# PKU-EPIC/HOTrack

Hardware: AMD Instinct MI355X
Metric: HandTrackNet point-cloud frames/sec (N=1024) (higher is better)
Workload: dtype f32; 1 GPU; HandTrackNet forward, batch=64 synthetic 1024-pt clouds per GPU (BASELINE configs[1]); per_gpu_batch=64, global_batch=64, npoints=1024, parallelism=dp1 (independent batches, no collective), world_size=1, resident_batches_rotated=5, dead_attention_elided=True, fused_sa_kernels=True, launch=hipGraph replay, batches_in_flight=4, hip_hw_queues=4, sa_compute_units=256, weights=deterministic random init (no checkpoint available offline)

## Files before the change

### hotrack_amd/csrc/sa_fused.hip

```cpp
#include <stdlib.h>

#include "pn2_common.h"
#include "../../include/pn2_ext.h"

#ifndef SA_PAD
#define SA_PAD 4
#endif

#ifndef SA_DEFER_EPILOGUE
#define SA_DEFER_EPILOGUE 0
#endif
#ifndef SA_OVERLAP_WRITEOUT
#define SA_OVERLAP_WRITEOUT 1
#endif
#ifndef SA_SCALAR_L1
#define SA_SCALAR_L1 0
#endif
#ifndef SA_LOADER_PRIO
#define SA_LOADER_PRIO 0
#endif
#ifndef SA_PROBE
#define SA_PROBE 0
#endif
#ifndef SA_PREFETCH
// ... 54 lines not shown
}

struct SaArgs {
    int B, N, S, K, lgK;
    const float *a1f;
    const float *xyz;
    const float *cxyz;
    const float *wx;
    const float *b1;
    const float *cadd;
    int a1f_ld, cadd_ld;
    const int *idx;
    const float *w2, *b2, *w3, *b3;
    const float *w2e;
    float *out;
    long out_b;
    int out_s, out_c;
    int num_tiles, tiles_per_cloud;
    long long *trace;
    const int *cls_list;
    const int *cls_sizes;
};

template <int C1, int C2, int C3, int WC, int RTC, int MINW, int NB1, int K, int MODE>
__device__ __forceinline__ void sa_body(const SaArgs &A, const int wg, const int nwg) {
    static_assert(K == 0 || K == 16 || K == 32 || K == 64, "K");
    constexpr bool CLS = K == 0;
    constexpr bool ROWS = MODE == 4 || MODE == 5, ROWS_EXTRA = MODE == 5;
    static_assert(!ROWS_EXTRA || SA_PAD >= 4, "the extra input columns live in the LDS row padding");
    constexpr bool has_a1f = MODE >= 1, has_xyz = !ROWS, has_cadd = MODE == 2 || MODE == 3;
    const bool p_a1f = MODE == 3 ? A.a1f != nullptr : has_a1f, p_xyz = MODE == 3 ? A.xyz != nullptr : has_xyz;
    const bool p_cadd = MODE == 3 ? A.cadd != nullptr : has_cadd;
    constexpr int lgK = K == 16 ? 4 : K == 32 ? 5 : 6;
    const int N = A.N, S = A.S;
    const float *__restrict__ W2 = A.w2, *__restrict__ b2 = A.b2, *__restrict__ W3 = A.w3, *__restrict__ b3 = A.b3;
    float *__restrict__ out = A.out;
    const int num_tiles = A.num_tiles, tiles_per_cloud = A.tiles_per_cloud;
    constexpr int WP = 4 / WC;
    constexpr int TM = WP * 64;
    constexpr int LD1 = C1 + SA_PAD, LD2 = C2 + SA_PAD;
    constexpr int NT2 = C2 / (16 * WC), NT3 = C3 / (16 * WC);
    static_assert(C2 % (16 * WC) == 0 && C3 % (16 * WC) == 0 && C1 % 16 == 0, "tile geometry");
    extern __shared__ __attribute__((aligned(16))) float smem[];
    float *H1ring = smem;
    float *H2 = smem + NB1 * TM * LD1;

    const int tid = (int)__builtin_amdgcn_workitem_id_x();
    const int lane = tid & 63;
    const int w = tid >> 6;
// ... 329 lines not shown
            }
#endif
            stamp(it, 4);
#if !(SA_PROBE & 2)
            if (nx.tile < end) finish(D1, H1n, 1);
#endif
            stamp(it, 5);
            __syncthreads();
            stamp(it, 6);
            nx = af;
            af = CLS ? ag : cursor_next(af);
            if constexpr (CLS) ag = cursor_next(ag);
        }
        return;
    }
#ifdef SA_COMPUTE_PRIO
    __builtin_amdgcn_s_setprio(SA_COMPUTE_PRIO);
#endif
    int it = 0;
    Cursor cc = cursor_at(first);
    constexpr int NP = 4 / RTC, NQ2 = C1 / 16, NQ3 = C2 / 16;
    constexpr int rstep = CLS ? 4 : K >> 4;
    const int oc_lane = (wc * NT3 + g) * 16 + li;
    const unsigned out_cloud = 4u * ((unsigned)(S - 1) * (unsigned)A.out_s + (unsigned)(C3 - 1) * (unsigned)A.out_c + 1u);
    const rsrc_t ro_rows = make_rsrc(out, ROWS ? 4u * (unsigned)N * (unsigned)A.out_s : 0u);
    float m[4][NT3];
#pragma unroll
    for (int rt = 0; rt < 4; ++rt)
#pragma unroll
        for (int ct = 0; ct < NT3; ++ct) m[rt][ct] = 0.f;
    int e_b = 0, e_pos0 = 0;
    bool e_pending = false;
    auto epilogue = [&]() {
        if constexpr (K == 32) {
#pragma unroll
            for (int ct = 0; ct < NT3; ++ct) {
                m[0][ct] = fmax_raw(m[0][ct], m[1][ct]);
                m[2][ct] = fmax_raw(m[2][ct], m[3][ct]);
            }
        }
        if constexpr (K == 64) {
#pragma unroll
            for (int ct = 0; ct < NT3; ++ct) m[0][ct] = fmax_raw(fmax3_raw(m[0][ct], m[1][ct], m[2][ct]), m[3][ct]);
        }
        const rsrc_t ro = make_rsrc(out + (size_t)e_b * A.out_b, e_pending ? out_cloud : 0u);
#pragma unroll
        for (int rt = 0; rt < 4; rt += rstep) {
            const int s = ((e_pos0 + wp * 64) >> lgK) + rt / rstep;
#pragma unroll
            for (int ct0 = 0; ct0 < NT3; ct0 += 4) {
                float v = rows_max4(m[rt][ct0]);
#pragma unroll
                for (int j = 1; j < 4; ++j)
                    if (ct0 + j < NT3) {
                        const float vj = rows_max4(m[rt][ct0 + j]);
                        v = g == j ? vj : v;
                    }
                const unsigned off = 4u * ((unsigned)s * (unsigned)A.out_s + (unsigned)(oc_lane + 16 * ct0) * (unsigned)A.out_c);
                const bool ok = ct0 + g < NT3 && s < S;
                __builtin_amdgcn_raw_buffer_store_b32(__builtin_bit_cast(unsigned, fmaxf(v, 0.f)), ro, (int)(ok ? off : 0xffffffffu), 0, 0);
            }
        }
    };
    int me_b = 0, me_s = 0;
    auto load_me = [&](const Cursor &cu) {
        const int lgk = 5 - cu.b;
        const int n_c = sel3(cu.b, cls_n0, cls_n1, cls_n2), off = sel3(cu.b, 0, cls_n0, cls_n0 + cls_n1);
        const rsrc_t rl = make_rsrc(A.cls_list + 4 * (size_t)off, 16u * (unsigned)n_c);
        const unsigned slot = ((unsigned)(cu.t * TM + wp * 64) >> lgk) + (unsigned)(lane & 7);
        const i32x2 v = __builtin_bit_cast(i32x2, __builtin_amdgcn_raw_buffer_load_b64(rl, (int)(16u * slot + 8u), 0, 0));
        me_b = v.x; me_s = v.y;
    };
    const unsigned out_all = 4u * ((unsigned)(A.B - 1) * (unsigned)A.out_b + (unsigned)(S - 1) * (unsigned)A.out_s + (unsigned)(C3 - 1) * (unsigned)A.out_c + 1u);
    auto epilogue_cls = [&](const Cursor &cu) {
        static_assert(!CLS || NT3 == 2, "class walk: a lane row stores one of two channel tiles");
        const int lgk = 5 - cu.b;
        const int n_c = sel3(cu.b, cls_n0, cls_n1, cls_n2);
        const int slot0 = (int)((unsigned)(cu.t * TM + wp * 64) >> lgk);
        const rsrc_t ro = make_rsrc(out, out_all);
        auto store = [&](float v, int src, int ct, bool lane_ok) {
            const unsigned bb = (unsigned)__builtin_amdgcn_ds_bpermute(4 * src, me_b), ss = (unsigned)__builtin_amdgcn_ds_bpermute(4 * src, me_s);
            const unsigned off = 4u * (bb * (unsigned)A.out_b + ss * (unsigned)A.out_s + (unsigned)((wc * NT3 + ct) * 16 + li) * (unsigned)A.out_c);
// ... 181 lines not shown

template <int C1, int C2, int C3, int WC, int RTC, int MINW, int NB1, int K, int MODE>
__global__ void __launch_bounds__(512, MINW)
sa_mlp_max_kernel(const SaArgs A, const int grid) {
    sa_body<C1, C2, C3, WC, RTC, MINW, NB1, K, MODE>(A, (int)__builtin_amdgcn_workgroup_id_x(), grid);
}

template <int C1, int C2, int C3, int WC, int RTC, int MINW, int NB1, int MODE>
__global__ void __launch_bounds__(512, MINW)
sa_mlp_max_classes_kernel(const SaArgs A, const int grid) {
    sa_body<C1, C2, C3, WC, RTC, MINW, NB1, 0, MODE>(A, (int)__builtin_amdgcn_workgroup_id_x(), grid);
}

template <int C1, int C2, int C3, int WC, int RTC, int MINW, int NB1, int K0, int K1, int MODE>
__global__ void __launch_bounds__(512, MINW)
sa_mlp_max_pair_kernel(const SaArgs A0, const SaArgs A1, const int n0, const int n1) {
    const int wg = (int)__builtin_amdgcn_workgroup_id_x();
    if (wg < n0)
        sa_body<C1, C2, C3, WC, RTC, MINW, NB1, K0, MODE>(A0, wg, n0);
    else
        sa_body<C1, C2, C3, WC, RTC, MINW, NB1, K1, MODE>(A1, wg - n0, n1);
}

static int g_sa_cus = -1;
static int sa_compute_units() {
    if (g_sa_cus < 0) {
        const char *e = getenv("PN2_SA_CUS");
        g_sa_cus = e ? atoi(e) : 0;
    }
    const int all = num_compute_units();
    return (g_sa_cus > 0 && g_sa_cus < all) ? g_sa_cus : all;
}

constexpr int sa_tile_rows(int WC) { return (4 / WC) * 64; }

static int sa_set_tiles(SaArgs &a, int tm) {
    a.tiles_per_cloud = (a.S * a.K + tm - 1) / tm;
    const long num_tiles = (long)a.B * a.tiles_per_cloud;
    if (num_tiles > 2147483647L) return PN2_ERANGE;
    a.num_tiles = (int)num_tiles;
    a.lgK = 0;
    while ((1 << a.lgK) < a.K) ++a.lgK;
    return PN2_OK;
}

static int sa_grid_rounds(int tiles, int max_wg) {
// ... 13 lines not shown
static int sa_grid_classes(long centroids, int tm, long max_wg) {
    const long most = (centroids * 32 + tm - 1) / tm + 2;
    return (int)(most < max_wg ? most : max_wg);
}

template <auto kfn, int C1, int C2, int WC, int MINW, int NB1>
static int sa_launch_shape(size_t &lds) {
    lds = (size_t)sa_tile_rows(WC) * (NB1 * (C1 + SA_PAD) + C2 + SA_PAD) * sizeof(float);
    static PerDeviceOnce raised;
    if (lds > 64 * 1024 && raised.first_use())
        (void)hipFuncSetAttribute((const void *)kfn, hipFuncAttributeMaxDynamicSharedMemorySize, (int)lds);
    const int wg_per_cu = (int)((160 * 1024) / lds) < MINW / 2 ? (int)((160 * 1024) / lds) : MINW / 2;
    return sa_compute_units() * (wg_per_cu < 1 ? 1 : wg_per_cu);
}

template <int C1, int C2, int C3, int WC, int RTC, int MINW, int NB1, int K, int MODE>
static int launch_sa_km(SaArgs a, hipStream_t st) {
    if (sa_set_tiles(a, sa_tile_rows(WC)) != PN2_OK) return PN2_ERANGE;
    constexpr auto kfn = sa_mlp_max_kernel<C1, C2, C3, WC, RTC, MINW, NB1, K, MODE>;
    size_t lds;
    const int max_wg = sa_launch_shape<kfn, C1, C2, WC, MINW, NB1>(lds);
    const int grid = sa_grid_rounds(a.num_tiles, max_wg);
    hipLaunchKernelGGL(kfn, dim3(grid), dim3(512), lds, st, a, grid);
    return check_launch();
}

template <int C1, int C2, int C3, int WC, int RTC, int MINW, int NB1, int MODE>
static int launch_sa_classes(SaArgs a, hipStream_t st) {
    a.lgK = 5; a.tiles_per_cloud = 1;
    constexpr auto kfn = sa_mlp_max_classes_kernel<C1, C2, C3, WC, RTC, MINW, NB1, MODE>;
    size_t lds;
    const int max_wg = sa_launch_shape<kfn, C1, C2, WC, MINW, NB1>(lds);
    const int grid = sa_grid_classes((long)a.B * a.S, sa_tile_rows(WC), max_wg);
    hipLaunchKernelGGL(kfn, dim3(grid), dim3(512), lds, st, a, grid);
    return check_launch();
}

template <int C1, int C2, int C3, int WC, int RTC, int MINW, int NB1, int K0, int K1, int MODE>
static int launch_sa_pair(SaArgs a0, SaArgs a1, hipStream_t st) {
    if (sa_set_tiles(a0, sa_tile_rows(WC)) != PN2_OK || sa_set_tiles(a1, sa_tile_rows(WC)) != PN2_OK ||
        (long)a0.num_tiles + a1.num_tiles > 2147483647L)
        return PN2_ERANGE;
    constexpr auto kfn = sa_mlp_max_pair_kernel<C1, C2, C3, WC, RTC, MINW, NB1, K0, K1, MODE>;
    size_t lds;
    const int max_wg = sa_launch_shape<kfn, C1, C2, WC, MINW, NB1>(lds);
    int n0, n1;
    sa_grid_pair(a0.num_tiles, a1.num_tiles, max_wg, n0, n1);
    hipLaunchKernelGGL(kfn, dim3(n0 + n1), dim3(512), lds, st, a0, a1, n0, n1);
    return check_launch();
}

static int sa_mode(const SaArgs &a) {
    const bool fa = a.a1f != nullptr, fx = a.xyz != nullptr, fc = a.cadd != nullptr;
    if (!fx || (fc && !fa)) return 3;
    return fa ? (fc ? 2 : 1) : 0;
}

template <int C1, int C2, int C3, int WC, int RTC, int MINW, int NB1, int K>
static int launch_sa_k(const SaArgs &a, hipStream_t st) {
    switch (sa_mode(a)) {
        case 0: return launch_sa_km<C1, C2, C3, WC, RTC, MINW, NB1, K, 0>(a, st);
        case 1: return launch_sa_km<C1, C2, C3, WC, RTC, MINW, NB1, K, 1>(a, st);
        case 2: return launch_sa_km<C1, C2, C3, WC, RTC, MINW, NB1, K, 2>(a, st);
    }
    return launch_sa_km<C1, C2, C3, WC, RTC, MINW, NB1, K, 3>(a, st);
}

template <int C1, int C2, int C3, int WC, int RTC, int MINW, int NB1>
static int launch_sa(const SaArgs &a, hipStream_t st) {
    switch (a.K) {
        case 16: return launch_sa_k<C1, C2, C3, WC, RTC, MINW, NB1, 16>(a, st);
// ... 219 lines not shown
}

extern "C" int pn2x_sa_mlp_max_pair_supported(int k0, int k1, int c1, int c2, int c3) {
    return (c1 == 128 && c2 == 128 && c3 == 192 && ((k0 == 16 && k1 == 64) || (k0 == 64 && k1 == 16))) ? 1 : 0;
}

static_assert(sizeof(pn2x_sa_problem) == 144, "record layout (pn2_ext.h)");
extern "C" int pn2x_sa_mlp_max_pair(int b, int c1, int c2, int c3, const pn2x_sa_problem *p0, const pn2x_sa_problem *p1, void *stream) {
    using namespace pn2;
    if (b < 0 || !p0 || !p1) return b < 0 ? PN2_EINVAL : PN2_ENULL;
    if (b == 0) return PN2_OK;
    if (!pn2x_sa_mlp_max_pair_supported(p0->k, p1->k, c1, c2, c3)) return PN2_ERANGE;
    if (p0->k > p1->k) { const pn2x_sa_problem *t = p0; p0 = p1; p1 = t; }
    SaArgs a0, a1;
    if (const int rc = sa_check_fill(b, *p0, c1, c3, a0); rc != PN2_OK) return rc;
    if (const int rc = sa_check_fill(b, *p1, c1, c3, a1); rc != PN2_OK) return rc;
    const int mode = sa_mode(a0);
    if (mode != sa_mode(a1) || (mode != 1 && mode != 2)) return PN2_ERANGE;
    hipStream_t st = (hipStream_t)stream;
    if (mode == 2) return launch_sa_pair<128, 128, 192, 4, SA_RTC128, 2, SA_NB1, 16, 64, 2>(a0, a1, st);
    return launch_sa_pair<128, 128, 192, 4, SA_RTC128, 2, SA_NB1, 16, 64, 1>(a0, a1, st);
}

extern "C" int pn2x_mlp2_rows_supported(int c1, int c2, int c3) { return (c1 == 128 && c2 == 128 && c3 == 128) ? 1 : 0; }

extern "C" int pn2x_mlp2_rows(long rows, int c1, int c2, int c3, const float *x, int ldx, const float *w2, const float *w2e, const float *b2,
                              const float *w3, const float *b3, float *out, int ldo, void *stream) {
    using namespace pn2;
    if (rows < 0 || ldx < c1 + (w2e ? 4 : 0) || ldo < c3 || ldx % 4 || ldo % 4) return PN2_EINVAL;
    if (rows == 0) return PN2_OK;
    if (!x || !w2 || !b2 || !w3 || !b3 || !out) return PN2_ENULL;
    if (!pn2x_mlp2_rows_supported(c1, c2, c3)) return PN2_ERANGE;
    if (((uintptr_t)x | (uintptr_t)w2 | (uintptr_t)w3 | (uintptr_t)out) % 16 != 0) return PN2_EINVAL;
    if (rows >= (1L << 24) - 64 || 4L * ldx >= (1L << 24) || 4L * rows * ldx > 0xffffffffL || 4L * rows * ldo > 0xffffffffL) return PN2_ERANGE;
    SaArgs a = {};
    a.B = 1; a.N = (int)rows; a.K = 16; a.S = (int)((rows + 15) / 16);
    a.a1f = x; a.a1f_ld = ldx; a.w2 = w2; a.b2 = b2; a.w3 = w3; a.b3 = b3; a.w2e = w2e; a.out = out; a.out_s = ldo; a.out_c = 1;
    if (w2e) return launch_sa_km<128, 128, 128, 4, 2, 2, SA_NB1, 16, 5>(a, (hipStream_t)stream);
    return launch_sa_km<128, 128, 128, 4, 2, 2, SA_NB1, 16, 4>(a, (hipStream_t)stream);
}

extern "C" int pn2x_sa_mlp_max_supported(int k, int c1, int c2, int c3) {
    const bool kk = (k == 16 || k == 32 || k == 64);
    const bool cc = (c1 == 32 && c2 == 32 && c3 == 64) || (c1 == 64 && c2 == 64 && c3 == 128) ||
                    (c1 == 128 && c2 == 128 && c3 == 192);
    return (kk && cc) ? 1 : 0;
// ... 2 lines not shown
```

### hotrack_amd/ext.py

```python
from __future__ import annotations

import ctypes
import os

import torch

from . import pointnet2_hip as _native

_lib = _native._lib
_vp, _ci = ctypes.c_void_p, ctypes.c_int
_lib.pn2x_kabsch.argtypes = [_ci, _ci, _ci, _vp, _vp, _vp, _vp, _vp]
_lib.pn2x_kabsch.restype = _ci


def kabsch(x: torch.Tensor, y: torch.Tensor):
    x = x.float().contiguous()
    y = y.float().contiguous()
    if x.dim() == 2:
        x = x.unsqueeze(0)
    B, num, _ = y.shape
    xb = x.shape[0]
    if xb not in (1, B) or x.shape[1] != num:
        raise ValueError(f"kabsch: x {tuple(x.shape)} does not match y {tuple(y.shape)}")
    px = _native._ptr(x, "x", torch.float32, xb * num * 3)
# ... 49 lines not shown
_lib.pn2x_three_nn_weights.restype = _ci
_lib.pn2x_three_interpolate_pm.argtypes = [_ci, _ci, _ci, _ci, _vp, _ci, _vp, _vp, _vp, _ci, _vp]
_lib.pn2x_three_interpolate_pm.restype = _ci
_lib.pn2x_gather_rows.argtypes = [_ci, _ci, _ci, _ci, _vp, _vp, _vp, _vp]
_lib.pn2x_gather_rows.restype = _ci
_lib.pn2x_bias_act_pm.argtypes = [_cl, _ci, _vp, _ci, _vp, _cl, _ci, _vp]
_lib.pn2x_bias_act_pm.restype = _ci


def sa_mlp_max_supported(k: int, c1: int, c2: int, c3: int) -> bool:
    return bool(_lib.pn2x_sa_mlp_max_supported(k, c1, c2, c3))


def _rows(t: torch.Tensor, name: str, cols: int):
    if not t.is_cuda or t.dtype != torch.float32 or t.dim() != 3:
        raise TypeError(f"{name}: expected a 3-D float32 GPU tensor")
    B, R, C = t.shape
    if C < cols or t.stride(2) != 1 or (R > 1 and B > 1 and t.stride(0) != R * t.stride(1)):
        raise ValueError(f"{name}: unsupported layout shape={tuple(t.shape)} strides={t.stride()}")
    return t.data_ptr(), t.stride(1)


def sa_mlp_max(idx: torch.Tensor, w2, b2, w3, b3, *, a1f=None, xyz=None, cxyz=None, wx=None, b1=None, cadd=None,
               out=None, point_major=False) -> torch.Tensor:
    return _sa_mlp_max(idx, w2, b2, w3, b3, None, a1f, xyz, cxyz, wx, b1, cadd, out, point_major)


_lib.pn2x_sa_mlp_max_classes.argtypes = [_ci] * 7 + [_vp, _ci, _vp, _vp, _vp, _vp, _vp, _ci, _vp, _vp, _vp, _vp, _vp, _vp, _vp, _vp, _cl, _ci, _ci, _vp]
_lib.pn2x_sa_mlp_max_classes.restype = _ci
_lib.pn2x_sa_mlp_max_classes_supported.argtypes = [_ci] * 4
_lib.pn2x_sa_mlp_max_classes_supported.restype = _ci
_lib.pn2x_sa_class_lists.argtypes = [_ci, _ci, _ci, _vp, _vp, _vp, _vp]
_lib.pn2x_sa_class_lists.restype = _ci
_lib.pn2x_sa_class_lists2.argtypes = [_ci, _ci, _ci, _vp, _vp, _vp] * 2 + [_vp]
_lib.pn2x_sa_class_lists2.restype = _ci


def sa_mlp_max_classes_supported(k: int, c1: int, c2: int, c3: int) -> bool:
    return bool(_lib.pn2x_sa_mlp_max_classes_supported(k, c1, c2, c3))


def sa_class_partition(counts: torch.Tensor):
    c = counts.reshape(-1)
    ids = torch.arange(c.numel(), dtype=torch.int32, device=c.device)
    masks = (c > 16, (c > 8) & (c <= 16), c <= 8)
    return torch.cat([ids[m] for m in masks]), torch.stack([m.sum() for m in masks]).to(torch.int32)

# ... 69 lines not shown
            _native._check(_native._call(_lib.pn2x_sa_mlp_max_classes, "sa_mlp_max_classes_kernel", None, B, N, S, K, C1, C2, C3, pa, lda,
                                         px, pcx, pwx, pb1, pc, ldc, pi, pl, ps, pw2, pb2, pw3, pb3, po, ob, os_, oc,
                                         _native._stream(idx)), "sa_mlp_max_classes")
        return out
    with torch.cuda.device(idx.device):
        _native._check(_native._call(_lib.pn2x_sa_mlp_max, "sa_mlp_max_kernel", None, B, N, S, K, C1, C2, C3, pa, lda, px, pcx,
                                     pwx, pb1, pc, ldc, pi, pw2, pb2, pw3, pb3, po, ob, os_, oc, _native._stream(idx)),
                       "sa_mlp_max")
    return out


class _SaProblem(ctypes.Structure):
    _fields_ = [("n", _ci), ("s", _ci), ("k", _ci), ("a1f", _vp), ("a1f_ld", _ci), ("xyz", _vp), ("cxyz", _vp), ("wx", _vp),
                ("b1", _vp), ("cadd", _vp), ("cadd_ld", _ci), ("idx", _vp), ("w2", _vp), ("b2", _vp), ("w3", _vp), ("b3", _vp),
                ("out", _vp), ("out_b", _cl), ("out_s", _ci), ("out_c", _ci)]


_lib.pn2x_sa_mlp_max_pair.argtypes = [_ci] * 4 + [ctypes.POINTER(_SaProblem)] * 2 + [_vp]
_lib.pn2x_sa_mlp_max_pair.restype = _ci
_lib.pn2x_sa_mlp_max_pair_supported.argtypes = [_ci] * 5
_lib.pn2x_sa_mlp_max_pair_supported.restype = _ci


def sa_mlp_max_pair(p0: dict, p1: dict) -> None:
    keys = ("idx", "w2", "b2", "w3", "b3", "a1f", "xyz", "cxyz", "wx", "b1", "cadd", "out")
    a = [{k: p.get(k) for k in keys} for p in (p0, p1)]
    C1, C2, C3 = a[0]["w2"].shape[1], a[0]["w2"].shape[0], a[0]["w3"].shape[0]
    same = all(tuple(a[1][k].shape) == tuple(a[0][k].shape) for k in ("w2", "w3"))
    modes = [(p["a1f"] is not None, p["xyz"] is not None, p["cadd"] is not None) for p in a]
    if not (same and modes[0] == modes[1] and modes[0][0] and modes[0][1]
            and _lib.pn2x_sa_mlp_max_pair_supported(a[0]["idx"].shape[2], a[1]["idx"].shape[2], C1, C2, C3)):
        for p in a:
            sa_mlp_max(p["idx"], p["w2"], p["b2"], p["w3"], p["b3"], a1f=p["a1f"], xyz=p["xyz"], cxyz=p["cxyz"], wx=p["wx"], b1=p["b1"],
                       cadd=p["cadd"], out=p["out"])
        return
    B = a[0]["idx"].shape[0]
    if a[0]["out"] is None or a[1]["out"] is None:
        raise TypeError("sa_mlp_max_pair: out is required")
    q0, q1 = (_sa_mlp_max(classes=None, point_major=False, record=True, **p) for p in a)
    with torch.cuda.device(a[0]["idx"].device):
        _native._check(_native._call(_lib.pn2x_sa_mlp_max_pair, "sa_mlp_max_pair_kernel", None, B, C1, C2, C3, ctypes.byref(q0),
                                     ctypes.byref(q1), _native._stream(a[0]["idx"])), "sa_mlp_max_pair")


_lib.pn2x_mlp2_rows.argtypes = [_cl] + [_ci] * 3 + [_vp, _ci, _vp, _vp, _vp, _vp, _vp, _vp, _ci, _vp]
_lib.pn2x_mlp2_rows.restype = _ci
_lib.pn2x_mlp2_rows_supported.argtypes = [_ci] * 3
_lib.pn2x_mlp2_rows_supported.restype = _ci


_lib.pn2x_sa_set_compute_units.argtypes = [_ci]
_lib.pn2x_sa_set_compute_units.restype = _ci


def sa_set_compute_units(n: int) -> None:
    _native._check(_lib.pn2x_sa_set_compute_units(int(n)), "sa_set_compute_units")


def mlp2_rows_supported(c1: int, c2: int, c3: int) -> bool:
    return bool(_lib.pn2x_mlp2_rows_supported(c1, c2, c3))


# ... 1248 lines not shown
```

### include/pn2_ext.h

```cpp
#ifndef PN2_EXT_H
#define PN2_EXT_H

#include "pn2_hip.h"

#ifdef __cplusplus
extern "C" {
#endif

int pn2x_kabsch(int b, int xb, int num, const float *x, const float *y, float *R, float *t, void *stream);
int pn2x_kabsch_backward(int b, int xb, int num, const float *x, const float *y, const float *R, const float *grad_R,
                         const float *grad_t, float *grad_y, void *stream);

int pn2x_hand_frame(int b, int xb, int num, int n, int j, const float *palm_template, const float *kp,
                    const int *palm_idx, const float *points, float scale, float *R, float *t, float *xyz2,
                    float *xyz1, float *xyz2_copy, int copy_ld, int *nonfinite, void *stream);

int pn2x_sa_mlp_max(int b, int n, int s, int k, int c1, int c2, int c3, const float *a1f, int a1f_ld,
                    const float *xyz, const float *cxyz, const float *wx, const float *b1, const float *cadd,
                    int cadd_ld, const int *idx,
                    const float *w2, const float *b2, const float *w3, const float *b3, float *out,
                    long out_b, int out_s, int out_c, void *stream);
int pn2x_sa_mlp_max_supported(int k, int c1, int c2, int c3);

int pn2x_sa_class_lists(int b, int s, int n, const int *counts, int *list, int *sizes, void *stream);
// ... 59 lines not shown

int pn2x_pose_head(int b, int j, int c, const float *h, const float *w, const float *bias, const float *xyz1,
                   const float *R, const float *t, float scale, float *kp_hand, float *kp_cam, const int *nonfinite,
                   void *stream);

typedef struct pn2x_sa_problem {
    int n, s, k;
    const float *a1f;
    int a1f_ld;
    const float *xyz, *cxyz, *wx, *b1, *cadd;
    int cadd_ld;
    const int *idx;
    const float *w2, *b2, *w3, *b3;
    float *out;
    long out_b;
    int out_s, out_c;
} pn2x_sa_problem;
int pn2x_sa_set_compute_units(int n);
int pn2x_mlp2_rows_supported(int c1, int c2, int c3);
int pn2x_mlp2_rows(long rows, int c1, int c2, int c3, const float *x, int ldx, const float *w2, const float *w2e, const float *b2,
                   const float *w3, const float *b3, float *out, int ldo, void *stream);
int pn2x_sa_mlp_max_pair_supported(int k0, int k1, int c1, int c2, int c3);
int pn2x_sa_mlp_max_pair(int b, int c1, int c2, int c3, const pn2x_sa_problem *p0, const pn2x_sa_problem *p1, void *stream);

int pn2x_row_lists(int b, int n, int j, int k_large, int k_small, const int *gi, const int *gi_small, int *list, int *counts,
                   void *stream);
int pn2x_row_chain_supported(int c_in, int c_h, int c_conv, int c_q);
int pn2x_row_chain(int b, int n, const float *x, int ldx, const int *list, const int *counts, const float *wa, const float *ba,
                   const float *wb, const float *bb, const float *wc, const float *bc, const float *wq, float *out, int ldo,
                   int grid, void *stream);

int pn2x_sa3_chain_supported(int s, int c_in, int c1, int c2, int c3);
int pn2x_sa3_chain(int b, int s, const float *x, int ldx, const float *w1, const float *b1, const float *w2, const float *b2,
                   const float *w3, const float *b3, float *part, void *stream);
int pn2x_fp3_chain_supported(int s, int c_l2, int c_l3, int c1, int c2);
int pn2x_fp3_chain(int b, int s, const float *x, int ldx, const float *part, const float *wgt, const float *bg, const float *wa,
                   const float *wf, const float *bf, float *out, int ldo, void *stream);

int pn2x_hand_shape_opt_supported(int p, int d, int t);
int pn2x_hand_shape_opt(int p, int d, int t, int iterations, const float *k0, const float *k, const float *pre,
                        const float *targets, const float *initial_scale, double scaling_coefficient2, double beta, float *out,
                        float *trace, void *stream);

typedef struct pn2x_hand_pose_setup {
    const int *parents, *pose_block, *skin_pack;
    const float *skin_w, *comps, *pre, *posedirs, *pose_mean;
// ... 265 lines not shown
```

### network/models/fast_eval.py

```python
from __future__ import annotations

import torch
import torch.nn.functional as F



def _lin_relu(x2d: torch.Tensor, W: torch.Tensor, b: torch.Tensor) -> torch.Tensor:
    from hotrack_amd import ext
    return ext.linear(x2d, W, b, relu=True)


def _lin(x2d: torch.Tensor, W: torch.Tensor, b: torch.Tensor = None) -> torch.Tensor:
    from hotrack_amd import ext
    return ext.linear(x2d, W, b)


class FastEval:
    MAX_POINTS = 16384

    def __init__(self, net):
        self.net = net
        self._shapes_seen = set()
        self._key = None
        self.P = None
        self._consts = {}
        self._idents = {}
        self.row_chain = True
        self.sa_classes = True

    def _palm_idx(self, device):
        key = ("palm", str(device))
        if key not in self._consts:
            self._consts[key] = torch.tensor([0, 1, 5, 9, 13, 17], dtype=torch.int32, device=device)
        return self._consts[key]

    def _scale(self, device):
        key = ("scale", str(device))
        if key not in self._consts:
            self._consts[key] = 0.2 * torch.ones(1, dtype=torch.float32, device=device)
        return self._consts[key]

    def _versions(self):
        return tuple((t._version, t.data_ptr(), t.device) for t in list(self.net.parameters()) + list(self.net.buffers()))

    @staticmethod
    def supported(net) -> bool:
        from hotrack_amd import ext
        bh = net.bhand
        if net.handframe != "kp" or not net.elide_dead_attention:
            return False

# ... 74 lines not shown
        P["wq_order"] = (i_s, 1 - i_s)
        P["wq"] = torch.cat([torch.cat([wq[i], wq[2 + i]], dim=0) for i in P["wq_order"]], dim=0)
        P["row_chain"] = None
        Wc = P["conv1"][0]
        if (len(fp1) == 2 and c_in == P["fp2"][-1][0].shape[0] and Ks[0] != Ks[1] and fp1[0][0].shape[1] == c_in + 3
                and ext.row_chain_supported(c_in, fp1[0][0].shape[0], Wc.shape[0], 4 * wq[0].shape[0])
                and fp1[1][0].shape == (c_in, c_in) and Wc.shape[1] == c_in and C == Wc.shape[0]):
            P["row_chain"] = dict(wa=ext.row_chain_pack(fp1[0][0]), ba=fp1[0][1].contiguous(),
                                  wb=ext.row_chain_pack(fp1[1][0]), bb=fp1[1][1].contiguous(),
                                  wc=ext.row_chain_pack(Wc), bc=P["conv1"][1].contiguous(), wq=ext.row_chain_pack(P["wq"]))
        P["mid_chain"] = None
        S2 = bh.sa2.npoint
        pf = P["fp3"]
        if (len(sa3) == 3 and len(pf["rest"]) == 1 and sa3[0][0].shape[1] == c_l2 + 3
                and ext.sa3_chain_supported(S2, c_l2, sa3[0][0].shape[0], sa3[1][0].shape[0], sa3[2][0].shape[0])
                and sa3[1][0].shape[1] == sa3[0][0].shape[0] and sa3[2][0].shape[1] == sa3[1][0].shape[0]
                and ext.fp3_chain_supported(S2, pf["wa"].shape[1], pf["wb"].shape[1], pf["wa"].shape[0], pf["rest"][0][0].shape[0])
                and pf["wb"].shape[1] == sa3[2][0].shape[0] and pf["rest"][0][0].shape[1] == pf["wa"].shape[0]):
            P["mid_chain"] = dict(sa3=[t for W, b in sa3 for t in (ext.row_chain_pack(W), b.contiguous())],
                                  wgt=pf["wb"].t().contiguous(), bg=pf["b"].contiguous(), wa=ext.row_chain_pack(pf["wa"]),
                                  wf=ext.row_chain_pack(pf["rest"][0][0]), bf=pf["rest"][0][1].contiguous())
        P["wc2"] = torch.cat([q[("q2", 0)]["wc"], q[("q2", 1)]["wc"]], dim=0).contiguous()
        P["head_w"] = net.final_mlp[2].weight.detach().squeeze(-1).contiguous()
        P["r1"] = (net.r1.linear.weight.detach().squeeze(-1), net.r1.linear.bias.detach(), net.r1._perm.t().contiguous())
        P["r2"] = (net.r2.linear.weight.detach().squeeze(-1), net.r2.linear.bias.detach(), net.r2._perm.t().contiguous())
        self.P, self._key = P, key
        return P

    def _large_batch(self, B, N) -> bool:
        from hotrack_amd import ext
        return self.row_chain and B * N >= 32768 and B <= ext.ROW_CHAIN_MAX_B

    def _perm_idx(self, perm, B):
        key = ("perm", B, str(perm.device))
        if key not in self._idents:
            self._idents[key] = perm.reshape(1, -1).to(torch.int32).expand(B, -1).contiguous()
        return self._idents[key]

    @staticmethod
    def _q_scales(ext, name, plan, q, xyz1, c1q, a_col, cadd, out, c_q):
        probs = []
        for i, (idx, a, nb_xyz) in enumerate(plan):
            p = q[(name, i)]
            probs.append(dict(idx=idx, w2=p["l2"][0], b2=p["l2"][1], w3=p["l3"][0], b3=p["l3"][1], a1f=a[:, :, a_col:a_col + c1q],
                              xyz=nb_xyz, cxyz=xyz1, wx=p["wx"], b1=p["b1"],
                              cadd=None if cadd is None else cadd[:, :, i * c1q:(i + 1) * c1q], out=out[:, :, i * c_q:(i + 1) * c_q]))
        if len(probs) == 2:
            ext.sa_mlp_max_pair(*probs)
        else:
            for p in probs:
                ext.sa_mlp_max(p.pop("idx"), p.pop("w2"), p.pop("b2"), p.pop("w3"), p.pop("b3"), **p)

    def forward(self, input, flag_dict):
        from hotrack_amd import gemm_tuning
        shape = tuple(input["hand_points"].shape[:2])
        first = shape not in self._shapes_seen
        self._shapes_seen.add(shape)
        with gemm_tuning.scope(tune=first):
            return self._forward(input, flag_dict)

    def _forward(self, input, flag_dict):
        G = self._geometry(input, flag_dict)
        return None if G is None else self._dense(G, flag_dict)

    def _geometry(self, input, flag_dict):
        from hotrack_amd import ext
        net = self.net
        P = self.prepare()
        if P is None:
            return None
        dev = net.device
        if flag_dict["track_flag"]:
# ... 111 lines not shown
        c1q = q[("q1", 0)]["l2"][0].shape[1]
        rc = P["row_chain"]
        if large and rc is not None and gi_small is not None:
            lst, counts = ext.row_lists(gi, gi_small, N)
            ext.three_nn_interpolate_pm(xyz2, l1_xyz, l1_out, fp1_in[:, :, :c_i], rows=(lst, counts))
            a_all = torch.empty((B, N, 4 * c1q), **f32)
            ext.row_chain(fp1_in, lst, counts, rc["wa"], rc["ba"], rc["wb"], rc["bb"], rc["wc"], rc["bc"], rc["wq"], out=a_all)
        else:
            ext.three_nn_interpolate_pm(xyz2, l1_xyz, l1_out, fp1_in[:, :, :c_i])
            f = P["fp1_fused"]
            if f is not None:
                x = ext.mlp2_rows(fp1_in.view(B * N, c_i + 4), f["w2"], f["b2"], f["w3"], f["b3"], w2e=f["w2e"])
            else:
                x = fp1_in.view(B * N, c_i + 4)[:, :c_i + 3]
                for W, b in P["fp1"]:
                    x = _lin_relu(x, W, b)
            src2 = _lin_relu(x, *P["conv1"])
            a_all = _lin(src2, P["wq"]).view(B, N, -1)
        plan = []
        for i, K in enumerate(Ks):
            j = P["wq_order"].index(i)
            idx = gi if K == kmax else (gi_small if K == kmin and gi_small is not None else gi[:, :, :K].contiguous())
            plan.append((idx, a_all[:, :, 2 * c1q * j:2 * c1q * (j + 1)], xyz2))
        f11 = torch.empty((B, J, 2 * c_q), **f32)
        self._q_scales(ext, "q1", plan, q, xyz1, c1q, 0, None, f11, c_q)
        Wr, br, perm = P["r1"]
        f12 = _lin(ext.gather_rows(f11, self._perm_idx(perm, B)).view(B * J, -1), Wr, br)
        cadd = _lin(f12, P["wc2"]).view(B, J, -1)
        f13 = torch.empty((B, J, 2 * c_q), **f32)
        self._q_scales(ext, "q2", plan, q, xyz1, c1q, c1q, cadd, f13, c_q)
        Wr, br, perm = P["r2"]
        f14 = _lin(ext.gather_rows(f13, self._perm_idx(perm, B)).view(B * J, -1), Wr, br)

        s11, c11, c3 = net.transt.s11, net.transt.c11, net.c3
        wf, bf = net.final_mlp[0].weight.squeeze(-1), net.final_mlp[0].bias
        if ext.ln_linear_supported(f14.shape[0], f14.shape[1]):
            x, hdn = ext.ln_linear(f14, s11.norm1, c11.linear1.weight, c11.linear1.bias, relu=True, ln2=c11.norm1)
            y = _lin(hdn, c11.linear2.weight)
            x, hdn = ext.ln_linear(x, c11.norm2, c3.linear1.weight, c3.linear1.bias, relu=True, y=y, ybias=c11.linear2.bias, ln2=c3.norm1)
            y = _lin(hdn, c3.linear2.weight)
            x, hdn = ext.ln_linear(x, c3.norm2, wf, bf, relu=True, y=y, ybias=c3.linear2.bias)
        else:
            x = ext.add_layernorm(f14, s11.norm1, ln2=c11.norm1)
            for blk, nxt in ((c11, c3.norm1), (c3, None)):
                hdn = _lin_relu(x, blk.linear1.weight, blk.linear1.bias)
                x = ext.add_layernorm(x, blk.norm2, y=_lin(hdn, blk.linear2.weight), bias=blk.linear2.bias, ln2=nxt)
            hdn = _lin_relu(x, wf, bf)
        pred_hf, pred_kp = ext.pose_head(hdn, P["head_w"], net.final_mlp[2].bias, xyz1, R, t, 0.2, nonfinite=nonfinite)

        ret = {"canon_pose": canon}
        ret["pred_kp_handframe"] = pred_hf.transpose(1, 2)
        ret["init_kp_handframe"] = xyz1.transpose(1, 2)
        ret["points_handframe"] = xyz2.transpose(1, 2)
        ret["pred_kp"] = pred_kp
        if flag_dict.get("IKNet_flag", False):
# ... 7 lines not shown
```

Baseline: 94550 frames/s.

## Scatter pooled SA outputs directly into permuted token rows, dropping gather_rows

Adds a destination-table variant of the fused SA MLP+maxpool kernels. The epilogue writes each pooled centroid row straight to every token row that the r1/r2 permutation maps it to, so the separate gather_rows kernel and its intermediate buffer are no longer needed. The table is built on the host once per weight set and passed by value as a kernel argument. In exchange the epilogue issues up to eight guarded stores per value and reads the per-centroid table from kernel-argument memory.

```diff
diff --git a/hotrack_amd/csrc/sa_fused.hip b/hotrack_amd/csrc/sa_fused.hip
--- a/hotrack_amd/csrc/sa_fused.hip
+++ b/hotrack_amd/csrc/sa_fused.hip
@@ -100,9 +100,17 @@
     const int *cls_sizes;
 };
 
-template <int C1, int C2, int C3, int WC, int RTC, int MINW, int NB1, int K, int MODE>
-__device__ __forceinline__ void sa_body(const SaArgs &A, const int wg, const int nwg) {
+constexpr int kDstMaxS = 64, kDstMaxPer = 8;
+struct alignas(16) SaDstRow { unsigned w[kDstMaxPer / 2]; };
+struct SaDst {
+    SaDstRow row[kDstMaxS];
+    int rows;
+};
+
+template <int C1, int C2, int C3, int WC, int RTC, int MINW, int NB1, int K, int MODE, bool DST = false>
+__device__ __forceinline__ void sa_body(const SaArgs &A, const int wg, const int nwg, const SaDst *__restrict__ T = nullptr) {
     static_assert(K == 0 || K == 16 || K == 32 || K == 64, "K");
+    static_assert(!DST || (K != 0 && MODE != 4 && MODE != 5), "a destination table goes with the fixed-K pooled epilogue only");
     constexpr bool CLS = K == 0;
     constexpr bool ROWS = MODE == 4 || MODE == 5, ROWS_EXTRA = MODE == 5;
     static_assert(!ROWS_EXTRA || SA_PAD >= 4, "the extra input columns live in the LDS row padding");
@@ -478,7 +486,7 @@
     constexpr int NP = 4 / RTC, NQ2 = C1 / 16, NQ3 = C2 / 16;
     constexpr int rstep = CLS ? 4 : K >> 4;
     const int oc_lane = (wc * NT3 + g) * 16 + li;
-    const unsigned out_cloud = 4u * ((unsigned)(S - 1) * (unsigned)A.out_s + (unsigned)(C3 - 1) * (unsigned)A.out_c + 1u);
+    const unsigned out_cloud = 4u * ((unsigned)((DST ? T->rows : S) - 1) * (unsigned)A.out_s + (unsigned)(C3 - 1) * (unsigned)A.out_c + 1u);
     const rsrc_t ro_rows = make_rsrc(out, ROWS ? 4u * (unsigned)N * (unsigned)A.out_s : 0u);
     float m[4][NT3];
 #pragma unroll
@@ -503,6 +511,8 @@
 #pragma unroll
         for (int rt = 0; rt < 4; rt += rstep) {
             const int s = ((e_pos0 + wp * 64) >> lgK) + rt / rstep;
+            SaDstRow q = {};
+            if constexpr (DST) q = T->row[__builtin_amdgcn_readfirstlane(s < S ? s : 0)];
 #pragma unroll
             for (int ct0 = 0; ct0 < NT3; ct0 += 4) {
                 float v = rows_max4(m[rt][ct0]);
@@ -514,6 +524,16 @@
                     }
                 const unsigned off = 4u * ((unsigned)s * (unsigned)A.out_s + (unsigned)(oc_lane + 16 * ct0) * (unsigned)A.out_c);
                 const bool ok = ct0 + g < NT3 && s < S;
+                if constexpr (DST) {
+                    const unsigned col = 4u * (unsigned)(oc_lane + 16 * ct0) * (unsigned)A.out_c;
+#pragma unroll
+                    for (int d = 0; d < kDstMaxPer; ++d) {
+                        const unsigned r = (q.w[d >> 1] >> (16 * (d & 1))) & 0xffffu;
+                        if (r != 0xffffu)
+                            __builtin_amdgcn_raw_buffer_store_b32(__builtin_bit_cast(unsigned, fmaxf(v, 0.f)), ro,
+                                                                  (int)(ok ? 4u * r * (unsigned)A.out_s + col : 0xffffffffu), 0, 0);
+                    }
+                } else
                 __builtin_amdgcn_raw_buffer_store_b32(__builtin_bit_cast(unsigned, fmaxf(v, 0.f)), ro, (int)(ok ? off : 0xffffffffu), 0, 0);
             }
         }
@@ -741,6 +761,22 @@
         sa_body<C1, C2, C3, WC, RTC, MINW, NB1, K1, MODE>(A1, wg - n0, n1);
 }
 
+template <int C1, int C2, int C3, int WC, int RTC, int MINW, int NB1, int K, int MODE>
+__global__ void __launch_bounds__(512, MINW)
+sa_mlp_max_dst_kernel(const SaArgs A, const int grid, const SaDst T) {
+    sa_body<C1, C2, C3, WC, RTC, MINW, NB1, K, MODE, true>(A, (int)__builtin_amdgcn_workgroup_id_x(), grid, &T);
+}
+
+template <int C1, int C2, int C3, int WC, int RTC, int MINW, int NB1, int K0, int K1, int MODE>
+__global__ void __launch_bounds__(512, MINW)
+sa_mlp_max_pair_dst_kernel(const SaArgs A0, const SaArgs A1, const int n0, const int n1, const SaDst T) {
+    const int wg = (int)__builtin_amdgcn_workgroup_id_x();
+    if (wg < n0)
+        sa_body<C1, C2, C3, WC, RTC, MINW, NB1, K0, MODE, true>(A0, wg, n0, &T);
+    else
+        sa_body<C1, C2, C3, WC, RTC, MINW, NB1, K1, MODE, true>(A1, wg - n0, n1, &T);
+}
+
 static int g_sa_cus = -1;
 static int sa_compute_units() {
     if (g_sa_cus < 0) {
@@ -800,6 +836,17 @@
     const int max_wg = sa_launch_shape<kfn, C1, C2, WC, MINW, NB1>(lds);
     const int grid = sa_grid_rounds(a.num_tiles, max_wg);
     hipLaunchKernelGGL(kfn, dim3(grid), dim3(512), lds, st, a, grid);
+    return check_launch();
+}
+
+template <int C1, int C2, int C3, int WC, int RTC, int MINW, int NB1, int K, int MODE>
+static int launch_sa_km_dst(SaArgs a, const SaDst &t, hipStream_t st) {
+    if (sa_set_tiles(a, sa_tile_rows(WC)) != PN2_OK) return PN2_ERANGE;
+    constexpr auto kfn = sa_mlp_max_dst_kernel<C1, C2, C3, WC, RTC, MINW, NB1, K, MODE>;
+    size_t lds;
+    const int max_wg = sa_launch_shape<kfn, C1, C2, WC, MINW, NB1>(lds);
+    const int grid = sa_grid_rounds(a.num_tiles, max_wg);
+    hipLaunchKernelGGL(kfn, dim3(grid), dim3(512), lds, st, a, grid, t);
     return check_launch();
 }
 
@@ -825,6 +872,20 @@
     int n0, n1;
     sa_grid_pair(a0.num_tiles, a1.num_tiles, max_wg, n0, n1);
     hipLaunchKernelGGL(kfn, dim3(n0 + n1), dim3(512), lds, st, a0, a1, n0, n1);
+    return check_launch();
+}
+
+template <int C1, int C2, int C3, int WC, int RTC, int MINW, int NB1, int K0, int K1, int MODE>
+static int launch_sa_pair_dst(SaArgs a0, SaArgs a1, const SaDst &t, hipStream_t st) {
+    if (sa_set_tiles(a0, sa_tile_rows(WC)) != PN2_OK || sa_set_tiles(a1, sa_tile_rows(WC)) != PN2_OK ||
+        (long)a0.num_tiles + a1.num_tiles > 2147483647L)
+        return PN2_ERANGE;
+    constexpr auto kfn = sa_mlp_max_pair_dst_kernel<C1, C2, C3, WC, RTC, MINW, NB1, K0, K1, MODE>;
+    size_t lds;
+    const int max_wg = sa_launch_shape<kfn, C1, C2, WC, MINW, NB1>(lds);
+    int n0, n1;
+    sa_grid_pair(a0.num_tiles, a1.num_tiles, max_wg, n0, n1);
+    hipLaunchKernelGGL(kfn, dim3(n0 + n1), dim3(512), lds, st, a0, a1, n0, n1, t);
     return check_launch();
 }
 
@@ -1090,6 +1151,68 @@
     return launch_sa_pair<128, 128, 192, 4, SA_RTC128, 2, SA_NB1, 16, 64, 1>(a0, a1, st);
 }
 
+namespace pn2 {
+static int sa_dst_fill(const pn2x_sa_dst &d, SaDst &t) {
+    if (!d.start || !d.row) return PN2_ENULL;
+    if (d.s < 1 || d.rows < 1) return PN2_EINVAL;
+    if (d.s > kDstMaxS || d.rows >= 0xffff) return PN2_ERANGE;
+    if (d.start[0] != 0) return PN2_EINVAL;
+    for (int s = 0; s < d.s; ++s)
+        if (d.start[s + 1] < d.start[s]) return PN2_EINVAL;
+    for (int s = 0; s < d.s; ++s)
+        if (d.start[s + 1] - d.start[s] > kDstMaxPer) return PN2_ERANGE;
+    for (int i = 0; i < d.start[d.s]; ++i)
+        if (d.row[i] < 0 || d.row[i] >= d.rows) return PN2_EINVAL;
+    t.rows = d.rows;
+    for (int s = 0; s < kDstMaxS; ++s) {
+        unsigned r[kDstMaxPer];
+        for (int j = 0; j < kDstMaxPer; ++j)
+            r[j] = (s < d.s && d.start[s] + j < d.start[s + 1]) ? (unsigned)d.row[d.start[s] + j] : 0xffffu;
+        for (int j = 0; j < kDstMaxPer / 2; ++j) t.row[s].w[j] = r[2 * j] | (r[2 * j + 1] << 16);
+    }
+    return PN2_OK;
+}
+
+static int sa_dst_problem_ok(const pn2x_sa_problem &p, const pn2x_sa_dst &d, int c3) {
+    if (p.s != d.s) return PN2_EINVAL;
+    if (4 * ((d.rows - 1L) * p.out_s + (c3 - 1L) * p.out_c + 1) >= 0xffffffffL) return PN2_ERANGE;
+    return PN2_OK;
+}
+}
+
+static_assert(sizeof(pn2x_sa_dst) == 24, "record layout (pn2_ext.h)");
+extern "C" int pn2x_sa_mlp_max_dst(int b, int c1, int c2, int c3, const pn2x_sa_problem *p0, const pn2x_sa_problem *p1,
+                                   const pn2x_sa_dst *dst, void *stream) {
+    using namespace pn2;
+    if (b < 0 || !p0 || !dst) return b < 0 ? PN2_EINVAL : PN2_ENULL;
+    if (b == 0) return PN2_OK;
+    if (!(c1 == 128 && c2 == 128 && c3 == 192)) return PN2_ERANGE;
+    if (p1 ? !pn2x_sa_mlp_max_pair_supported(p0->k, p1->k, c1, c2, c3) : (p0->k != 16 && p0->k != 64)) return PN2_ERANGE;
+    if (p1 && p0->k > p1->k) { const pn2x_sa_problem *t = p0; p0 = p1; p1 = t; }
+    SaArgs a0, a1;
+    if (const int rc = sa_check_fill(b, *p0, c1, c3, a0); rc != PN2_OK) return rc;
+    if (p1)
+        if (const int rc = sa_check_fill(b, *p1, c1, c3, a1); rc != PN2_OK) return rc;
+    const int mode = sa_mode(a0);
+    if ((p1 && mode != sa_mode(a1)) || (mode != 1 && mode != 2)) return PN2_ERANGE;
+    SaDst t;
+    if (const int rc = sa_dst_fill(*dst, t); rc != PN2_OK) return rc;
+    if (const int rc = sa_dst_problem_ok(*p0, *dst, c3); rc != PN2_OK) return rc;
+    if (p1)
+        if (const int rc = sa_dst_problem_ok(*p1, *dst, c3); rc != PN2_OK) return rc;
+    hipStream_t st = (hipStream_t)stream;
+    if (p1) {
+        if (mode == 2) return launch_sa_pair_dst<128, 128, 192, 4, SA_RTC128, 2, SA_NB1, 16, 64, 2>(a0, a1, t, st);
+        return launch_sa_pair_dst<128, 128, 192, 4, SA_RTC128, 2, SA_NB1, 16, 64, 1>(a0, a1, t, st);
+    }
+    if (a0.K == 16) {
+        if (mode == 2) return launch_sa_km_dst<128, 128, 192, 4, SA_RTC128, 2, SA_NB1, 16, 2>(a0, t, st);
+        return launch_sa_km_dst<128, 128, 192, 4, SA_RTC128, 2, SA_NB1, 16, 1>(a0, t, st);
+    }
+    if (mode == 2) return launch_sa_km_dst<128, 128, 192, 4, SA_RTC128, 2, SA_NB1, 64, 2>(a0, t, st);
+    return launch_sa_km_dst<128, 128, 192, 4, SA_RTC128, 2, SA_NB1, 64, 1>(a0, t, st);
+}
+
 extern "C" int pn2x_mlp2_rows_supported(int c1, int c2, int c3) { return (c1 == 128 && c2 == 128 && c3 == 128) ? 1 : 0; }
 
 extern "C" int pn2x_mlp2_rows(long rows, int c1, int c2, int c3, const float *x, int ldx, const float *w2, const float *w2e, const float *b2,
diff --git a/hotrack_amd/ext.py b/hotrack_amd/ext.py
--- a/hotrack_amd/ext.py
+++ b/hotrack_amd/ext.py
@@ -95,7 +95,13 @@
 
 
 def sa_mlp_max(idx: torch.Tensor, w2, b2, w3, b3, *, a1f=None, xyz=None, cxyz=None, wx=None, b1=None, cadd=None,
-               out=None, point_major=False) -> torch.Tensor:
+               out=None, point_major=False, dst=None) -> torch.Tensor:
+    if dst is not None:
+        if out is None:
+            raise TypeError("sa_mlp_max: dst needs out")
+        q = _sa_mlp_max(idx, w2, b2, w3, b3, None, a1f, xyz, cxyz, wx, b1, cadd, out, False, record=True)
+        _sa_launch_dst(idx, w2, w3, q, None, dst, out, "sa_mlp_max")
+        return out
     return _sa_mlp_max(idx, w2, b2, w3, b3, None, a1f, xyz, cxyz, wx, b1, cadd, out, point_major)
 
 
@@ -211,7 +217,36 @@
 _lib.pn2x_sa_mlp_max_pair_supported.restype = _ci
 
 
-def sa_mlp_max_pair(p0: dict, p1: dict) -> None:
+def sa_mlp_max_pair_supported(k0: int, k1: int, c1: int, c2: int, c3: int) -> bool:
+    return bool(_lib.pn2x_sa_mlp_max_pair_supported(k0, k1, c1, c2, c3))
+
+
+class _SaDst(ctypes.Structure):
+    _fields_ = [("start", _vp), ("row", _vp), ("s", _ci), ("rows", _ci)]
+
+
+_lib.pn2x_sa_mlp_max_dst.argtypes = [_ci] * 4 + [ctypes.POINTER(_SaProblem)] * 2 + [ctypes.POINTER(_SaDst), _vp]
+_lib.pn2x_sa_mlp_max_dst.restype = _ci
+
+
+def _sa_launch_dst(idx, w2, w3, q0, q1, dst, out, what):
+    if not (isinstance(dst, (tuple, list)) and len(dst) == 2):
+        raise TypeError(f"{what}: dst must be the (dst_start, dst_row) pair")
+    start, row = dst
+    for name, t in (("dst_start", start), ("dst_row", row)):
+        if not isinstance(t, torch.Tensor) or t.is_cuda or t.dtype != torch.int32 or t.dim() != 1 or not t.is_contiguous():
+            raise TypeError(f"{what}: {name} must be a contiguous 1-D int32 CPU tensor")
+    B, S = idx.shape[0], idx.shape[1]
+    if start.numel() != S + 1 or int(start[-1]) != row.numel():
+        raise ValueError(f"{what}: dst_start needs S + 1 = {S + 1} entries, the last one the length of dst_row")
+    d = _SaDst(start.data_ptr(), row.data_ptr() if row.numel() else None, S, out.shape[1])
+    with torch.cuda.device(idx.device):
+        _native._check(_native._call(_lib.pn2x_sa_mlp_max_dst, "sa_mlp_max_pair_dst_kernel" if q1 is not None else "sa_mlp_max_dst_kernel",
+                                     None, B, w2.shape[1], w2.shape[0], w3.shape[0], ctypes.byref(q0),
+                                     None if q1 is None else ctypes.byref(q1), ctypes.byref(d), _native._stream(idx)), what)
+
+
+def sa_mlp_max_pair(p0: dict, p1: dict, dst=None) -> None:
     keys = ("idx", "w2", "b2", "w3", "b3", "a1f", "xyz", "cxyz", "wx", "b1", "cadd", "out")
     a = [{k: p.get(k) for k in keys} for p in (p0, p1)]
     C1, C2, C3 = a[0]["w2"].shape[1], a[0]["w2"].shape[0], a[0]["w3"].shape[0]
@@ -221,12 +256,15 @@
             and _lib.pn2x_sa_mlp_max_pair_supported(a[0]["idx"].shape[2], a[1]["idx"].shape[2], C1, C2, C3)):
         for p in a:
             sa_mlp_max(p["idx"], p["w2"], p["b2"], p["w3"], p["b3"], a1f=p["a1f"], xyz=p["xyz"], cxyz=p["cxyz"], wx=p["wx"], b1=p["b1"],
-                       cadd=p["cadd"], out=p["out"])
+                       cadd=p["cadd"], out=p["out"], dst=dst)
         return
     B = a[0]["idx"].shape[0]
     if a[0]["out"] is None or a[1]["out"] is None:
         raise TypeError("sa_mlp_max_pair: out is required")
     q0, q1 = (_sa_mlp_max(classes=None, point_major=False, record=True, **p) for p in a)
+    if dst is not None:
+        _sa_launch_dst(a[0]["idx"], a[0]["w2"], a[0]["w3"], q0, q1, dst, a[0]["out"], "sa_mlp_max_pair")
+        return
     with torch.cuda.device(a[0]["idx"].device):
         _native._check(_native._call(_lib.pn2x_sa_mlp_max_pair, "sa_mlp_max_pair_kernel", None, B, C1, C2, C3, ctypes.byref(q0),
                                      ctypes.byref(q1), _native._stream(a[0]["idx"])), "sa_mlp_max_pair")
diff --git a/include/pn2_ext.h b/include/pn2_ext.h
--- a/include/pn2_ext.h
+++ b/include/pn2_ext.h
@@ -105,6 +105,14 @@
                    const float *w3, const float *b3, float *out, int ldo, void *stream);
 int pn2x_sa_mlp_max_pair_supported(int k0, int k1, int c1, int c2, int c3);
 int pn2x_sa_mlp_max_pair(int b, int c1, int c2, int c3, const pn2x_sa_problem *p0, const pn2x_sa_problem *p1, void *stream);
+struct pn2x_sa_dst {
+    const int *start;
+    const int *row;
+    int s, rows;
+};
+typedef struct pn2x_sa_dst pn2x_sa_dst;
+int pn2x_sa_mlp_max_dst(int b, int c1, int c2, int c3, const pn2x_sa_problem *p0, const pn2x_sa_problem *p1, const pn2x_sa_dst *dst,
+                        void *stream);
 
 int pn2x_row_lists(int b, int n, int j, int k_large, int k_small, const int *gi, const int *gi_small, int *list, int *counts,
                    void *stream);
diff --git a/network/models/fast_eval.py b/network/models/fast_eval.py
--- a/network/models/fast_eval.py
+++ b/network/models/fast_eval.py
@@ -27,6 +27,7 @@
         self._idents = {}
         self.row_chain = True
         self.sa_classes = True
+        self.scatter_tokens = True
 
     def _palm_idx(self, device):
         key = ("palm", str(device))
@@ -147,14 +148,26 @@
                                   wf=ext.row_chain_pack(pf["rest"][0][0]), bf=pf["rest"][0][1].contiguous())
         P["wc2"] = torch.cat([q[("q2", 0)]["wc"], q[("q2", 1)]["wc"]], dim=0).contiguous()
         P["head_w"] = net.final_mlp[2].weight.detach().squeeze(-1).contiguous()
-        P["r1"] = (net.r1.linear.weight.detach().squeeze(-1), net.r1.linear.bias.detach(), net.r1._perm.t().contiguous())
-        P["r2"] = (net.r2.linear.weight.detach().squeeze(-1), net.r2.linear.bias.detach(), net.r2._perm.t().contiguous())
+        for name, mod in (("r1", net.r1), ("r2", net.r2)):
+            perm = mod._perm.t().contiguous()
+            P[name] = (mod.linear.weight.detach().squeeze(-1), mod.linear.bias.detach(), perm, self._token_table(perm))
         self.P, self._key = P, key
         return P
 
     def _large_batch(self, B, N) -> bool:
         from hotrack_amd import ext
         return self.row_chain and B * N >= 32768 and B <= ext.ROW_CHAIN_MAX_B
+
+    @staticmethod
+    def _token_table(perm):
+        src = perm.reshape(-1).cpu().to(torch.int64)
+        J = perm.shape[0]
+        counts = torch.bincount(src, minlength=J)
+        if J > 64 or int(counts.max()) > 8:
+            return None
+        start = torch.zeros(J + 1, dtype=torch.int32)
+        start[1:] = torch.cumsum(counts, 0).to(torch.int32)
+        return start, torch.argsort(src, stable=True).to(torch.int32).contiguous()
 
     def _perm_idx(self, perm, B):
         key = ("perm", B, str(perm.device))
@@ -163,7 +176,7 @@
         return self._idents[key]
 
     @staticmethod
-    def _q_scales(ext, name, plan, q, xyz1, c1q, a_col, cadd, out, c_q):
+    def _q_scales(ext, name, plan, q, xyz1, c1q, a_col, cadd, out, c_q, dst=None):
         probs = []
         for i, (idx, a, nb_xyz) in enumerate(plan):
             p = q[(name, i)]
@@ -171,8 +184,9 @@
                               xyz=nb_xyz, cxyz=xyz1, wx=p["wx"], b1=p["b1"],
                               cadd=None if cadd is None else cadd[:, :, i * c1q:(i + 1) * c1q], out=out[:, :, i * c_q:(i + 1) * c_q]))
         if len(probs) == 2:
-            ext.sa_mlp_max_pair(*probs)
-        else:
+            ext.sa_mlp_max_pair(*probs, dst=dst)
+        else:
+            assert dst is None
             for p in probs:
                 ext.sa_mlp_max(p.pop("idx"), p.pop("w2"), p.pop("b2"), p.pop("w3"), p.pop("b3"), **p)
 
@@ -330,15 +344,23 @@
             j = P["wq_order"].index(i)
             idx = gi if K == kmax else (gi_small if K == kmin and gi_small is not None else gi[:, :, :K].contiguous())
             plan.append((idx, a_all[:, :, 2 * c1q * j:2 * c1q * (j + 1)], xyz2))
-        f11 = torch.empty((B, J, 2 * c_q), **f32)
-        self._q_scales(ext, "q1", plan, q, xyz1, c1q, 0, None, f11, c_q)
-        Wr, br, perm = P["r1"]
-        f12 = _lin(ext.gather_rows(f11, self._perm_idx(perm, B)).view(B * J, -1), Wr, br)
+        Ksq = [q[("q1", i)]["K"] for i in range(2)]
+        pair_ok = self.scatter_tokens and len(plan) == 2 and ext.sa_mlp_max_pair_supported(Ksq[0], Ksq[1], c1q, q[("q1", 0)]["l2"][0].shape[0], c_q)
+
+        def q_tokens(name, a_col, cadd, r):
+            Wr, br, perm, table = P[r]
+            if pair_ok and table is not None:
+                tok = torch.empty((B, perm.numel(), 2 * c_q), **f32)
+                self._q_scales(ext, name, plan, q, xyz1, c1q, a_col, cadd, tok, c_q, dst=table)
+            else:
+                f = torch.empty((B, J, 2 * c_q), **f32)
+                self._q_scales(ext, name, plan, q, xyz1, c1q, a_col, cadd, f, c_q)
+                tok = ext.gather_rows(f, self._perm_idx(perm, B))
+            return _lin(tok.view(B * J, -1), Wr, br)
+
+        f12 = q_tokens("q1", 0, None, "r1")
         cadd = _lin(f12, P["wc2"]).view(B, J, -1)
-        f13 = torch.empty((B, J, 2 * c_q), **f32)
-        self._q_scales(ext, "q2", plan, q, xyz1, c1q, c1q, cadd, f13, c_q)
-        Wr, br, perm = P["r2"]
-        f14 = _lin(ext.gather_rows(f13, self._perm_idx(perm, B)).view(B * J, -1), Wr, br)
+        f14 = q_tokens("q2", c1q, cadd, "r2")
 
         s11, c11, c3 = net.transt.s11, net.transt.c11, net.c3
         wf, bf = net.final_mlp[0].weight.squeeze(-1), net.final_mlp[0].bias
```

Measured after the change: 94820 frames/s (median of 6 runs). No clear change (+0.3%).
